# ajzhai/PEANUT

Hardware: AMD Instinct MI355X
Metric: maps/sec for 480x480x(4+N_cat) prediction fwd, batch 32 (higher is better)
Workload: dtype f32; 1 GPU; 480x480, 14-channel (4+10) partial maps -> 6-class prediction forward (PSPNet R50-V1c-D8), batch 32 per GPU, seeded random-init weights; survey_config=2, global_batch=32, parallelism=dp1 (map shards, no data-path collective)

## Files before the change

peanut_amd/csrc/common.h:

```cpp
#pragma once
#include <hip/hip_runtime.h>
#include <stdint.h>
#include <string>

namespace peanut {

void set_error(const std::string& msg);
int fail(int code, const std::string& msg);
void note_kernel(const char* family);
const char* noted_kernel();

#define PEANUT_HIP_CHECK(expr)                                                            \
  do {                                                                                    \
    hipError_t _e = (expr);                                                               \
    if (_e != hipSuccess)                                                                 \
      return ::peanut::fail(-3, std::string(#expr) + ": " + hipGetErrorString(_e));       \
  } while (0)

struct ConvDesc {
  int cin;
  int cout;
  int kh, kw, stride, pad, dil;
  int relu;
  int bn_tile;
// ... 74 lines not shown
bool conv_pw_uses_256w(int cout, long long M, int mt_per_group, int bn_tile, int cin, int flush_ktiles);
bool conv_pw_narrow_tiles(int cin, int cout, long long M, int bn_tile, int mt_per_group);
bool conv_pw_uses_256p(int cout, long long M, int mt_per_group, int bn_tile, int cin, int flush_ktiles, long long in_pixels = 0);
struct ConvKParams;
bool gemm_skinny_takes(const ConvKParams& p, int bn_tile, size_t ws_floats);
int launch_gemm_skinny(const ConvKParams& p, float* ws, size_t ws_floats, hipStream_t stream);
bool conv_pw_uses_256wp(int cout, long long M, int stride, int mt_per_group, int bn_tile, int c1, int c2, int flush_ktiles);
bool conv_pw_uses_ares(int cin, int cout, long long M, int stride, bool two_source, int flush_ktiles, int bn_tile);

bool conv_patch_eligible(const ConvDesc& d, const ConvArgs& a);
const char* conv_patch_kernel_name(const ConvDesc& d, bool nchw);
bool conv_patch_nchw_eligible(const ConvDesc& d, int B, int Ho, int Wo, int creal);
int launch_conv_patch_nchw(const ConvDesc& d, const float* x_nchw, int creal, float* y, int B, int H, int W, int Ho, int Wo, hipStream_t stream);

void wino_geometry(int B, int H, int W, int dil, int* th, int* tw, long long* n_tiles, long long* m_pad, int gran = 128, int m = 4);
void wino_transform_weights(const float* w_oihw, int cout, int cin, float* out, int m = 4);
int launch_wino_input(const float* x, float* V, int B, int H, int W, int C, int dil, hipStream_t s, int gran = 128, int m = 4, long long m_pad_total = 0,
                      const DeferredSplit* df = nullptr);
bool wino_input_accepts_deferred(int B, int H, int W, int C, int dil, int gran, int m);
long long wino_deferred_count();
int launch_wino_output(const float* Mb, const float* scale, const float* shift, const float* res, float* y,
                       int B, int H, int W, int C, int dil, int relu, hipStream_t s, int gran = 128, int m = 4, long long m_pad_total = 0);

bool gemm_rs_uses_256(int cout, long long M, int mt_per_group, int bn_tile, int cin);
const char* gemm_rs_kernel_name(int cout, long long M, int mt_per_group, int bn_tile, int cin, int planes);
size_t sx_packed_bytes(int cin_pad, int cout, int bn_tile, int planes);
void pack_weights_sx(const float* w, int cout, int cin_real, int cin_pad, int bn_tile, int planes, float wscale, void* out);
float sx_pack_scale(const float* w, size_t n, int planes);
size_t sx_conv_packed_bytes(int cin_pad, int cout, int kh, int kw, int bn_tile, int planes);
void pack_weights_sx_conv(const float* w_oihw, int cout, int cin_real, int cin_pad, int kh, int kw, int bn_tile, int planes,
                          float wscale, void* out);

int launch_nchw_to_nhwc_pad(const float* x, float* y, int B, int C, int H, int W, int Cpad, hipStream_t s);
int launch_maxpool3x3s2(const float* x, float* y, int B, int H, int W, int C, int Ho, int Wo, hipStream_t s);
int launch_ppm_pool(const float* x, float* out, int B, int H, int W, int C, const int* scales, int nscales,
                    hipStream_t s, int scale_rows = 0);
size_t ppm_pool_scratch_floats(int B, int H, int C, const int* scales, int nscales);
int launch_ppm_pool2(const float* x, float* scratch, float* out, int B, int H, int W, int C, const int* scales,
                     int nscales, hipStream_t s, int scale_rows = 0);
int launch_ppm_upsample_concat(const float* table, float* out, int B, int H, int W, int Cp, const int* scales,
                               int nscales, int align_corners, hipStream_t s);
int launch_ppm_conv_term(const float* Q, float* R, int B, int H, int W, int C, const int* scales, int nscales,
                         int align_corners, hipStream_t s, int scale_rows = 0);
int launch_upsample_logits(const float* lo, float* out, int B, int h, int w, int K, int H, int W,
                           int align_corners, int sigmoid, hipStream_t s);

// ... 2 lines not shown
```

peanut_amd/csrc/net_common.h:

```cpp
#pragma once
#include <stdlib.h>
#include <math.h>

#include <stdint.h>

#include <map>
#include <memory>
#include <string>
#include <vector>

#include "../../include/peanut_hip.h"
#include "common.h"
#include "options.h"

namespace peanut {

struct DevBuf {
  void* p = nullptr;
  size_t bytes = 0;
  ~DevBuf() { if (p) (void)hipFree(p); }
  int ensure(size_t n) {
    if (n <= bytes) return 0;
    if (p) { (void)hipFree(p); p = nullptr; bytes = 0; }
    hipError_t e = hipMalloc(&p, n);
// ... 43 lines not shown
      if (e2 != hipSuccess) { (void)hipGraphDestroy(g); return fail(PEANUT_EHIP, std::string("hipGraphInstantiate: ") + hipGetErrorString(e2)); }
      hit->graph = g;
      hit->exec = x;
    }
    PEANUT_HIP_CHECK(hipGraphLaunch(hit->exec, s));
    return 0;
  }
};

struct ConvLayer {
  std::string name;
  ConvDesc d{};
  int cin_real = 0;
  DevBuf w, ss;
  bool has_wino = false;
  ConvDesc wino{};
  size_t wino_group_floats = 0;
  DevBuf wino_w, wino_ss;
  DevBuf w_s, wino_w_s;
  size_t wino_group_bytes = 0;
  int wino_m = 4;
  int wino_np() const { return (wino_m + 2) * (wino_m + 2); }
  std::unique_ptr<ConvLayer> alt;
};

inline int rs_planes_of(int precision) {
  return precision == PEANUT_PREC_BF16X6 ? 3 : (precision == PEANUT_PREC_BF16X3 ? 2 : (precision == PEANUT_PREC_FP16X3 ? 4 : 0));
}
inline bool precision_known(int precision) { return precision == PEANUT_PREC_FP32 || rs_planes_of(precision) != 0; }
inline int precision_of_planes(int planes) {
  return planes == 3 ? PEANUT_PREC_BF16X6 : (planes == 2 ? PEANUT_PREC_BF16X3 : (planes == 4 ? PEANUT_PREC_FP16X3 : PEANUT_PREC_FP32));
}
inline bool rs_conv_enabled() {
  return opt(OPT_RS_CONV) != 0;
}
inline int rs_bn_tile(int cin_pad, int cout, int kh, int kw, int pad) {
  if (kh != 1 || kw != 1 || pad != 0 || cin_pad % 16 != 0 || cout < 64) return 0;
  const int bn64_maxk = (int)opt(OPT_RS_BN64_MAXK);
  return (cout >= 128 && cin_pad > bn64_maxk) ? 128 : 64;
}

inline int upload_conv(ConvLayer& L, const float* w_oihw, const float* scale, const float* shift, int cout, int cin,
                int cin_pad, int kh, int kw, int stride, int pad, int dil, int relu, int precision) {
  if (cin_pad % 16 != 0 || cin_pad < cin) return fail(PEANUT_EINVAL, L.name + ": cin_pad must be a multiple of 16 and >= cin");
  ConvDesc& d = L.d;
  d.cin = cin_pad; d.cout = cout; d.kh = kh; d.kw = kw; d.stride = stride; d.pad = pad; d.dil = dil; d.relu = relu;
// ... 117 lines not shown
  g.scale = (const float*)L.wino_ss.p;
  g.shift = (const float*)L.wino_ss.p + g.cout_pad;
  L.wino_group_floats = gf;
  if (g.rs) {
    const size_t gb = sx_packed_bytes(cin_pad, cout, g.bn_tile, g.s_planes);
    std::vector<unsigned char> ps((size_t)np * gb);
    const float wscale = sx_pack_scale(U.data(), U.size(), g.s_planes);
    g.s_alpha = 1.f / wscale;
    for (int pos = 0; pos < np; ++pos)
      pack_weights_sx(U.data() + (size_t)pos * cout * cin, cout, cin, cin_pad, g.bn_tile, g.s_planes, wscale, ps.data() + pos * gb);
    if ((rc = L.wino_w_s.ensure(ps.size()))) return rc;
    PEANUT_HIP_CHECK(hipMemcpy(L.wino_w_s.p, ps.data(), ps.size(), hipMemcpyHostToDevice));
    g.w_s = L.wino_w_s.p;
    L.wino_group_bytes = gb;
  }
  L.has_wino = true;
  return 0;
}

inline int upload_wino_forms(ConvLayer& L, const float* w_oihw, const float* scale, const float* shift, int cout, int cin,
                             int cin_pad, int pad, int dil, int relu, int precision, int requested) {
  int rc;
  if ((rc = upload_wino(L, w_oihw, cout, cin, cin_pad, precision, requested))) return rc;
  if (requested != 0 || L.wino_m != 6) return 0;
  L.alt = std::make_unique<ConvLayer>();
  L.alt->name = L.name;
  if ((rc = upload_conv(*L.alt, w_oihw, scale, shift, cout, cin, cin_pad, 3, 3, 1, pad, dil, relu, precision)) ||
      (rc = upload_wino(*L.alt, w_oihw, cout, cin, cin_pad, precision, 4)))
    return rc;
  if (L.alt->wino_m != 4) { L.alt.reset(); return 0; }
  if (wino5_wanted(dil)) {
    auto& A5 = L.alt->alt;
    A5 = std::make_unique<ConvLayer>();
    A5->name = L.name;
    if ((rc = upload_conv(*A5, w_oihw, scale, shift, cout, cin, cin_pad, 3, 3, 1, pad, dil, relu, precision)) ||
        (rc = upload_wino(*A5, w_oihw, cout, cin, cin_pad, precision, 5)))
      return rc;
  }
  return 0;
}

inline int wino_gran_for(const ConvLayer& L, int B, int H, int W) {
  int th, tw;
  long long n_tiles, m_pad;
  wino_geometry(B, H, W, L.d.dil, &th, &tw, &n_tiles, &m_pad, 256, L.wino_m);
  {
// ... 9 lines not shown
             ? 256 : 128;
}

inline long long wino_padded_rows(const ConvLayer& L, int B, int H, int W) {
  int th, tw;
  long long n_tiles, m_pad;
  wino_geometry(B, H, W, L.d.dil, &th, &tw, &n_tiles, &m_pad, wino_gran_for(L, B, H, W), L.wino_m);
  return (long long)L.wino_np() * m_pad;
}

inline const ConvLayer* wino_pick_form(const ConvLayer* L, int B, int H, int W) {
  if (!L->has_wino || !L->alt || !L->alt->has_wino) return L;
  const ConvLayer* f4 = nullptr;
  const ConvLayer* big = nullptr;
  long long big_rows = 0;
  for (const ConvLayer* c = L; c && c->has_wino; c = c->alt.get()) {
    if (c->wino_m == 4) { f4 = c; continue; }
    const long long r = wino_padded_rows(*c, B, H, W);
    if (!big || r < big_rows || (r == big_rows && c->wino_m < big->wino_m)) { big = c; big_rows = r; }
  }
  if (!f4) return big ? big : L;
  if (!big) return f4;
  return big_rows * 10 <= wino_padded_rows(*f4, B, H, W) * 9 ? big : f4;
}

inline void wino_scratch_floats(const ConvLayer& L, int B, int H, int W, size_t* v, size_t* m) {
  int th, tw;
  long long n_tiles, m_pad;
  wino_geometry(B, H, W, L.d.dil, &th, &tw, &n_tiles, &m_pad, wino_gran_for(L, B, H, W), L.wino_m);
  *v = (size_t)L.wino_np() * m_pad * L.d.cin;
  *m = (size_t)L.wino_np() * m_pad * L.d.cout;
}

inline bool conv_layer_accepts_deferred(const ConvLayer& L, int B, int H, int W) {
  if (!L.has_wino || L.d.rs || L.wino.rs) return false;
  return wino_input_accepts_deferred(B, H, W, L.d.cin, L.d.dil, wino_gran_for(L, B, H, W), L.wino_m);
}

inline int launch_conv_layer(const ConvLayer& L, const ConvArgs& a, float* wino_v, float* wino_m, hipStream_t s, DeferredSplit* produced = nullptr) {
  const bool deferred_in = produced && produced->valid;
  if (!(L.has_wino && !a.x2 && wino_v && wino_m)) {
    if (deferred_in) return fail(PEANUT_EINVAL, L.name + ": the producer deferred its split-K reduce to a layer that cannot sum it");
    return launch_conv(L.d, a, s);
  }
  int th, tw, rc;
  long long n_tiles, m_pad;
// ... 106 lines not shown
```

peanut_amd/csrc/options.h:

```cpp
#pragma once
#include <stdlib.h>
#include <string.h>

#include <string>

namespace peanut {

enum OptionId {
  OPT_PW_GLDS, OPT_PW256_MINK, OPT_PW256_MINTILES, OPT_PW256_PHASE, OPT_PW256_SKIP_PAD, OPT_PW256W_MINK, OPT_PW256W_MINTILES, OPT_PW256P_MINK, OPT_PW256P_MINTILES, OPT_PW256P_FLUSH, OPT_PW256P_ORDER, OPT_PW256P_STREAMK, OPT_PW256WP_MINK, OPT_PW256WP_MINTILES, OPT_PW256WP_NPRE, OPT_PW256WP_STAGGER, OPT_PW_ARES, OPT_PW_SKINNY,
  OPT_PW_ARES_MINUNITS, OPT_PATCH_MINTILES, OPT_STEM_NCHW, OPT_BN64_MAXK, OPT_PW_BN64_MAXK, OPT_PW64_MAXTILES, OPT_FP32_BK, OPT_NCHUNK, OPT_RES_PREFETCH, OPT_SPLIT_MODEL,
  OPT_RS_CONV, OPT_RS_BN64_MAXK, OPT_RS256_MINK, OPT_RS256_MINTILES, OPT_RS64_MAXK, OPT_RS64_MAXTILES,
  OPT_WINO_M, OPT_WINO_HEAD_M, OPT_WINO6_MAXDIL, OPT_WINO5_MINDIL, OPT_WINO_FLUSH_CH, OPT_WINO_MIN_CIN, OPT_WINO_NARROW_MINPIX, OPT_WINO_SMALL_MAXWG, OPT_DEFER_SPLITK,
  OPT_PPM_OVERLAP, OPT_PPM_GROUPED, OPT_PPM_TERM_ROWS, OPT_PPM_GROUP_ROWS, OPT_RCNN_WINO_M, OPT_RCNN_STEM_S2D, OPT_RCNN_RPN_FUSED, OPT_RCNN_FPN_OVERLAP, OPT_RCNN_RANK_SORT, OPT_RCNN_TOPK_SLICE, OPT_RCNN_NMS_LEVELS, OPT_FMM_LOCAL32, OPT_FMM_MAX_PASSES, OPT_FMM_BLOCKED, OPT_FMM_INNER,
  OPT_COUNT
};

struct OptionInfo {
  const char* key;
  long long def;
  bool upload_time;
  const char* help;
};

inline const OptionInfo* option_table() {
  static const OptionInfo t[OPT_COUNT] = {
      {"pw_glds", 1, false, "fp32 1x1 convs / grouped GEMMs on the LDS-DMA kernels of conv_pw.hip (0: conv_igemm)"},
      {"pw256_mink", 1024, false, "fewest input channels for the 256 x 128 three-stage kernel"},
      {"pw256_mintiles", 256, false, "fewest 256 x 128 tiles for that kernel"},
      {"pw256_phase", 1, false, "the two waves of a SIMD request their LDS-DMA pieces half an iteration apart"},
      {"pw256_skip_pad", 1, false, "256 x 128 kernel, grouped GEMMs: waves whose rows are all group padding issue no MFMAs (0: compute the zero rows)"},
      {"pw256w_mink", 768, false, "fewest input channels for the 256 x 256 two-stage kernel (0: off)"},
      {"pw256w_mintiles", 1536, false, "fewest 256 x 256 tiles for that kernel"},
      {"pw256p_mink", 512, false, "fewest input channels for the persistent 256 x 128 kernel (conv_pw256p.hip; 0: off)"},
      {"pw256p_mintiles", 512, false, "fewest 256 x 128 tiles for that kernel"},
      {"pw256p_flush", 512, false, "most input channels of a Winograd position GEMM (two-level accumulation) that runs on the persistent kernel (0: none)"},
// ... 9 lines not shown
      {"patch_mintiles", 1024, false, "3x3 convs of 16 / 32 input channels on the persistent LDS-patch kernel (conv_patch.hip) from this many 8 x 16 output tiles (0: off)"},
      {"stem_nchw", 1, false, "prediction forward: the first stem conv reads the NCHW input itself (conv_patch.hip, NCHW variant) instead of a layout pass + NHWC conv (fp32 mode, when the patch kernel takes the layer)"},
      {"bn64_maxk", 256, true, "128 x 64 tiles for layers with at most this many input channels"},
      {"pw_bn64_maxk", 128, true, "pointwise layers / Winograd position GEMMs: weights PACKED 64 wide up to this many input channels (wider layers: 128-wide packing, 64-wide tiles chosen per shape)"},
      {"pw64_maxtiles", 512, false, "a 128-wide-packed pointwise layer with at most bn64_maxk input channels runs 128 x 64 tiles while its 128 x 128 tiling has fewer tiles than this (two per CU)"},
      {"fp32_bk", 0, true, "16: force 16-channel k-tiles in conv_igemm (experiment)"},
      {"nchunk", 8, false, "n-tiles per chunk of the tile order (0: n fastest over all n-tiles)"},
      {"res_prefetch", 1, false, "request the first residual rows before the last k-tile's MFMAs"},
      {"split_model", 1, false, "tail split-K plan counts CUs (1) or resident slots (0)"},
      {"rs_conv", 1, true, "emulated modes: non-pointwise convs on conv_rs.hip (0: fp32 MFMA kernel)"},
      {"rs_bn64_maxk", 128, true, "emulated modes: 128 x 64 tiles up to this many input channels"},
      {"rs256_mink", 512, false, "emulated modes: fewest input channels for the 256 x 256 kernel"},
      {"rs256_mintiles", 256, false, "emulated modes: fewest 256 x 256 tiles for it"},
      {"rs64_maxk", 512, false, "emulated modes: 64 x 64 tiles up to this many input channels"},
      {"rs64_maxtiles", 128, false, "emulated modes: ... and below this many 128-row tiles"},
      {"wino_m", 0, true, "4 / 5 / 6: force one Winograd form on every eligible layer (0: policy)"},
      {"wino_head_m", 0, true, "4 / 5 / 6: Winograd form of the PSP bottleneck (0: policy)"},
      {"wino6_maxdil", 4, true, "largest dilation that gets an F(6x6) form"},
      {"wino5_mindil", 4, true, "smallest dilation that also gets an F(5x5) form (0: none)"},
      {"wino_flush_ch", 64, true, "channels per partial sum of the position GEMMs' two-level accumulation (0: off)"},
      {"wino_min_cin", 0, true, "fewest input channels of a Winograd layer (0: the planner's policy)"},
      {"wino_narrow_minpix", 20000, false, "layers under 128 channels take their Winograd form from this many input pixels on (round 6: 100 000 -> 20 000 -- with the small-problem transforms one 720 x 720 map's layer1 conv2, 32 400 pixels, gains 5 us per layer as F(6x6); profiles/r9e)"},
      {"wino_small_maxwg", 1024, false, "Winograd transforms: launches with fewer workgroups than this of the one-thread-per-tile kernels take the small-problem variants (a workgroup per tile and 64-channel slice, a thread per line, through LDS; bit-identical; 0: never)"},
      {"defer_splitk", 1, false, "a Bottleneck conv1 whose every tile is split along k leaves its partial tiles unsummed and conv2's (small-problem) Winograd input transform sums them: one launch fewer per block at batch 1, bit-identical (0: every conv runs its own reduce); read when a (B, H, W) plan is built"},
      {"ppm_overlap", -1, false, "pyramid branch of the PSP head on a side stream: 0 / 1, -1 = by size"},
      {"ppm_grouped", -1, false, "per-scale PSP GEMMs as one grouped launch: 0 / 1, -1 = by size"},
      {"ppm_term_rows", 1, false, "folded pyramid term: one wave per output row, no barrier in the row loop (0: the workgroup-wide two-phase kernel)"},
      {"ppm_group_rows", 0, false, "pyramid pooling, row pass: rows added up per workgroup (1..5; 0 = by size: as many as still leave ~768 workgroups)"},
      {"rcnn_wino_m", 0, true, "detector front end: 4 / 5 / 6 pins one Winograd form (0: per shape)"},
      {"rcnn_stem_s2d", 1, true, "detector stem 7x7 stride 2 as a space-to-depth 4x4 conv"},
      {"rcnn_rpn_fused", 1, false, "detector: the RPN head on all five pyramid levels as one chain (five input transforms, ONE grouped Winograd GEMM, five output transforms, one objectness and one anchor-delta GEMM over all levels' rows: 12 launches instead of 25); read when a (B, H, W) plan is built"},
      {"rcnn_fpn_overlap", 0, false, "detector: the FPN output convs of p5, p4, p3 on a side stream next to the lateral / top-down chain that ends in p2's (round 5 experiment, bit-identical; measured SLOWER at batch 1, 5.70 against 5.61 ms per frame, profiles/r8: off); read when a (B, H, W) plan is built"},
      {"rcnn_rank_sort", 1, false, "detector: the RPN candidates of an image are ordered by counting the larger keys (n / 64 workgroups) instead of one workgroup's bitonic sort (round 5; same order: the keys are distinct)"},
      {"rcnn_topk_slice", 20480, false, "detector: objectness logits per workgroup of the per-level top-k (a level is cut into up to 8 ranges whose k largest are merged by counting; 0: one workgroup per level, round 4)"},
      {"rcnn_nms_levels", 1, false, "detector: the proposal NMS level by level (five 16 x 16-word suppression blocks and five scans per image side by side, post-NMS top-k by counting) instead of one score-sorted list per image (round 5; same proposals)"},
      {"fmm_local32", 1, false, "goal solver: single-precision local solve inside a tile"},
      {"fmm_max_passes", 24, false, "goal solver: hard ceiling of the second-order ordering passes; they stop as soon as a pass changes nothing (6-10 passes on the agent's 960 x 960 map; peanut_goal_converged reports whether they reached their fixed point)"},
      {"fmm_blocked", 1, false, "goal solver: a wave relaxes its 8 x 8 block of the tile to convergence between workgroup barriers (round 5; 0: one Jacobi sweep of the whole tile per barrier pair)"},
      {"fmm_inner", 48, false, "goal solver: iterations a wave spends on its block before it publishes it (blocked rounds)"},
  };
  return t;
}

struct Options {
  long long v[OPT_COUNT];
};
// ... 48 lines not shown
```

peanut_amd/csrc/pred_api.hip:

```cpp
#include <math.h>
#include <string.h>

#include <map>
#include <memory>
#include <string>
#include <vector>

#include "net_common.h"

namespace peanut {

static thread_local std::string g_err;
void set_error(const std::string& msg) { g_err = msg; }
int fail(int code, const std::string& msg) {
  g_err = msg;
  return code;
}
static thread_local const char* g_kernel = "";
void note_kernel(const char* family) { g_kernel = family; }
const char* noted_kernel() { return g_kernel; }

namespace {

enum OpKind { OP_TO_NHWC, OP_CONV, OP_CONV_NCHW, OP_MAXPOOL, OP_PPM_POOL, OP_PPM_UP, OP_PPM_TERM, OP_UPSAMPLE, OP_WINO_IN, OP_WINO_GEMM, OP_WINO_OUT };

struct Op {
  OpKind kind;
  std::string name;
  std::string kernel;
  const ConvLayer* conv = nullptr;
  Act in, in2, res, out;
  bool has_in2 = false, has_res = false;
  double flops = 0;
  double bytes = 0;
  int wino_mt_per_group = 0;
  int wino_valid_rows = 0;
  int wino_gran = 128;
  int branch = 0;
  bool fork_before = false, join_before = false;
  int group_mt = 0;
  int ppm_scale_rows = 0;
  bool defer_ok = false;
};

struct Plan {
  int B = 0, H = 0, W = 0;
  Act splitk;
// ... 149 lines not shown
    a.B = out->B; a.Ho = out->H; a.Wo = out->W;
    if (conv_patch_eligible(d, a)) return conv_patch_kernel_name(d, false);
  }
  if (d.rs == 2) return std::string(d.s_planes == 3 ? "conv_rs6_128x" : (d.s_planes == 4 ? "conv_rs3h_128x" : "conv_rs3_128x")) + std::to_string(d.bn_tile);
  if (d.rs) return gemm_rs_kernel_name(d.cout, M, mt_per_group, d.bn_tile, d.cin, d.s_planes);
  if (d.bk == 32 && d.kh == 1 && d.kw == 1 && d.pad == 0 && (!two_source || d.stride == 1) && d.cin % 32 == 0 && conv_pw_enabled())
  {
    const int flush = d.flush_ch / d.bk;
    if (conv_pw_uses_256wp(d.cout, M, d.stride, mt_per_group, d.bn_tile, d.cin, 0, flush))
      return "conv_pw_glds_256x256p";
    if (conv_pw_uses_ares(d.cin, d.cout, M, d.stride, two_source, flush, d.bn_tile)) return "conv_pw_ares_128x128";
    if (conv_pw_uses_256w(d.cout, M, mt_per_group, d.bn_tile, d.cin, flush)) return "conv_pw_glds_256x256";
    if (conv_pw_uses_256p(d.cout, M, mt_per_group, d.bn_tile, d.cin, flush, M * d.stride * d.stride)) return "conv_pw_glds_256x128p";
    if (conv_pw_uses_256(d.cout, M, mt_per_group, d.bn_tile, d.cin)) return "conv_pw_glds_256x128";
    if (conv_pw_narrow_tiles(d.cin, d.cout, M, d.bn_tile, mt_per_group)) return "conv_pw_glds_128x64";
    return "conv_pw_glds_128x" + std::to_string(d.bn_tile);
  }
  return "conv_igemm_128x" + std::to_string(d.bn_tile) + "x" + std::to_string(d.bk);
}

void push_conv(Plan& pl, const ConvLayer* L, const Act& in, const Act* in2, const Act* res, const Act& out, Arena* ar = nullptr) {
  const bool wino = L->has_wino && !in2 && ar && (long long)in.B * in.H * in.W >= wino_min_pixels(L->d.cin);
  if (wino) L = wino_pick_form(L, in.B, in.H, in.W);
  if (wino) {
    int th, tw;
    long long n_tiles, m_pad;
    const bool rs_gemm = L->wino.rs != 0;
    const int gran = wino_gran_for(*L, in.B, in.H, in.W);
    wino_geometry(in.B, in.H, in.W, L->d.dil, &th, &tw, &n_tiles, &m_pad, gran, L->wino_m);
    const double np = (double)L->wino_np();
    const long long npl = L->wino_np();
    Act v = make_act(*ar, 1, 1, (int)(npl * m_pad), in.C);
    Act m = make_act(*ar, 1, 1, (int)(npl * m_pad), L->d.cout);
    const std::string fam = L->wino_m == 6 ? "wino6_" : (L->wino_m == 5 ? "wino5_" : "wino_");
    const std::string tag = "[" + fam;
    Op a; a.kind = OP_WINO_IN; a.name = L->name + tag + "in]"; a.kernel = fam + "input"; a.conv = L; a.in = in; a.out = v;
    a.wino_gran = gran;
    a.bytes = (double)in.bytes + np * (double)n_tiles * in.C * 4.0;
    pl.ops.push_back(a);
    Op g; g.kind = OP_WINO_GEMM; g.name = L->name + tag + "gemm]"; g.kernel = conv_kernel_name(L->wino, false, npl * m_pad, (int)(m_pad / 128)); g.conv = L;
    g.in = v; g.in.W = (int)(npl * m_pad); g.in.C = in.C; g.out = m; g.wino_mt_per_group = (int)(m_pad / 128); g.wino_gran = gran; g.wino_valid_rows = (int)n_tiles;
    g.flops = 2.0 * np * (double)m_pad * L->d.cout * L->cin_real;
    g.bytes = np * (double)m_pad * (in.C * 4.0 + L->d.cout * 4.0) +
              np * (rs_gemm ? (double)L->wino_group_bytes : (double)L->wino_group_floats * 4);
    pl.ops.push_back(g);
    Op o; o.kind = OP_WINO_OUT; o.name = L->name + tag + "out]"; o.kernel = fam + "output"; o.conv = L; o.in = m; o.out = out;
// ... 61 lines not shown
    Act y = make_act(ar, B, conv_out_dim(x.H, 3, 2, 1, 1), conv_out_dim(x.W, 3, 2, 1, 1), x.C);
    Op op; op.kind = OP_MAXPOOL; op.name = "maxpool"; op.kernel = "maxpool"; op.in = x; op.out = y;
    op.bytes = (double)x.bytes + (double)y.bytes;
    pl->ops.push_back(op);
    pl->named["pool"] = y;
    rel(x);
    x = y;
  }
  for (size_t li = 0; li < h->layers.size(); ++li) {
    for (size_t bi = 0; bi < h->layers[li].size(); ++bi) {
      const auto& blk = h->layers[li][bi];
      const ConvDesc& d2 = blk.c2->d;
      Act t1 = make_act(ar, B, x.H, x.W, blk.c1->d.cout);
      push_conv(*pl, blk.c1, x, nullptr, nullptr, t1);
      const int h2 = conv_out_dim(x.H, 3, d2.stride, d2.pad, d2.dil), w2 = conv_out_dim(x.W, 3, d2.stride, d2.pad, d2.dil);
      Act t2 = make_act(ar, B, h2, w2, d2.cout);
      const size_t c1_idx = pl->ops.size() - 1;
      push_conv(*pl, blk.c2, t1, nullptr, nullptr, t2, &ar);
      {
        const Op& win = pl->ops[c1_idx + 1];
        if (opt(OPT_DEFER_SPLITK) != 0 && !h->keep_all && win.kind == OP_WINO_IN && pl->ops[c1_idx].kind == OP_CONV && !win.conv->d.rs &&
            wino_input_accepts_deferred(t1.B, t1.H, t1.W, t1.C, win.conv->d.dil, win.wino_gran, win.conv->wino_m))
          pl->ops[c1_idx].defer_ok = true;
      }
      rel(t1);
      Act idn = x;
      bool own_idn = false;
      const bool fused_c3d = blk.c3d != nullptr && !h->keep_all;
      if (blk.down && !fused_c3d) {
        idn = make_act(ar, B, h2, w2, blk.down->d.cout);
        push_conv(*pl, blk.down, x, nullptr, nullptr, idn);
        own_idn = true;
      }
      Act y = make_act(ar, B, h2, w2, blk.c3->d.cout);
      if (fused_c3d) push_conv(*pl, blk.c3d, t2, &x, nullptr, y);
      else push_conv(*pl, blk.c3, t2, nullptr, &idn, y);
      rel(t2);
      if (own_idn) rel(idn);
      rel(x);
      x = y;
    }
    pl->named["layer" + std::to_string(li + 1)] = x;
  }
  const int overlap_env = (int)opt(OPT_PPM_OVERLAP);
  const bool overlap = h->bottleneck_x != nullptr && (overlap_env >= 0 ? overlap_env == 1 : (long long)B * x.H * x.W >= 4096);
  const size_t side_first = pl->ops.size();
// ... 185 lines not shown
      }
      if (op.defer_ok) a.defer = &h->deferred;
      return launch_conv(op.conv->d, a, s);
    }
    case OP_WINO_IN: {
      const int rc = launch_wino_input(P(op.in), P(op.out), op.in.B, op.in.H, op.in.W, op.in.C, op.conv->d.dil, s, op.wino_gran, op.conv->wino_m, 0,
                                       h->deferred.valid ? &h->deferred : nullptr);
      h->deferred.valid = false;
      return rc;
    }
    case OP_WINO_GEMM: {
      ConvArgs a{};
      a.x = P(op.in); a.y = P(op.out);
      a.B = 1; a.H = 1; a.W = op.in.W; a.c1 = op.in.C; a.c2 = 0; a.Ho = 1; a.Wo = op.in.W;
      a.ws = P(op.branch ? pl.splitk2 : pl.splitk); a.ws_floats = kSplitKScratchFloats;
      a.mt_per_group = op.wino_mt_per_group;
      a.group_valid_rows = op.wino_valid_rows;
      a.w_group_stride = op.conv->wino.rs ? op.conv->wino_group_bytes : op.conv->wino_group_floats;
      return launch_conv(op.conv->wino, a, s);
    }
    case OP_WINO_OUT:
      return launch_wino_output(P(op.in), op.conv->d.scale, op.conv->d.shift, op.has_res ? P(op.res) : nullptr, P(op.out),
                                op.out.B, op.out.H, op.out.W, op.out.C, op.conv->d.dil, op.conv->d.relu, s, op.wino_gran, op.conv->wino_m);
    case OP_MAXPOOL:
      return launch_maxpool3x3s2(P(op.in), P(op.out), op.in.B, op.in.H, op.in.W, op.in.C, op.out.H, op.out.W, s);
    case OP_PPM_POOL:
      return launch_ppm_pool2(P(op.in), op.has_in2 ? P(op.in2) : nullptr, P(op.out), op.in.B, op.in.H, op.in.W, op.in.C,
                              h->cfg.pool_scales, h->cfg.n_pool_scales, s, op.ppm_scale_rows);
    case OP_PPM_UP:
      return launch_ppm_upsample_concat(P(op.in), P(op.out), op.out.B, op.out.H, op.out.W, h->cfg.head_channels,
                                        h->cfg.pool_scales, h->cfg.n_pool_scales, h->cfg.align_corners, s);
    case OP_PPM_TERM:
      return launch_ppm_conv_term(P(op.in), P(op.out), op.out.B, op.out.H, op.out.W, h->cfg.head_channels,
                                  h->cfg.pool_scales, h->cfg.n_pool_scales, h->cfg.align_corners, s, op.ppm_scale_rows);
    case OP_UPSAMPLE:
      return launch_upsample_logits(P(op.in), out_dev, op.in.B, op.in.H, op.in.W, op.in.C, pl.H, pl.W,
                                    h->cfg.align_corners, sigmoid, s);
  }
  return fail(PEANUT_EINVAL, "unknown op");
}

extern "C" {

const char* peanut_last_error(void) { return g_err.c_str(); }
const char* peanut_last_conv_kernel(void) { return noted_kernel(); }
int peanut_abi_version(void) { return 15; }
// ... 389 lines not shown
```

peanut_amd/csrc/winograd.hip:

```cpp
#include <stdlib.h>

#include <atomic>

#include "common.h"
#include "conv_common.h"

namespace peanut {

namespace {

template <typename V>
__device__ __forceinline__ V fmak(V a, float k, V c) { return __builtin_elementwise_fma(a, (V)k, c); }

__device__ __forceinline__ void bt6(const f32x4 d0, const f32x4 d1, const f32x4 d2, const f32x4 d3, const f32x4 d4,
                                    const f32x4 d5, f32x4& t0, f32x4& t1, f32x4& t2, f32x4& t3, f32x4& t4, f32x4& t5) {
#pragma clang fp contract(off)
  const f32x4 a = fmak(d2, -2.25f, d4), b = fmak(d3, 0.75f, -1.6875f * d1);
  const f32x4 c = fmak(d2, -0.5625f, d4), e = fmak(d3, 1.5f, -0.84375f * d1);
  t0 = fmak(d0, 1.265625f, fmak(d2, -2.8125f, d4));
  t1 = a + b;
  t2 = a - b;
  t3 = c + e;
  t4 = c - e;
  t5 = fmak(d1, 1.265625f, fmak(d3, -2.8125f, d5));
// ... 630 lines not shown
#pragma unroll
    for (int k = 0; k < 4; ++k) {
      const int r = r0 + k * g.d;
      const bool ok = c < g.W && r < g.H;
      const size_t off = ok ? (img + (size_t)r * g.W + c) * g.C + ng * 4 : 0;
      rc[k] = *reinterpret_cast<const f32x4*>(res + off);
    }
  }
  const f32x4 sc = *reinterpret_cast<const f32x4*>(scale + ng * 4);
  const f32x4 sh = *reinterpret_cast<const f32x4*>(shift + ng * 4);
  f32x4 o0, o1, o2, o3;
  at6(qs[0][a][l], qs[1][a][l], qs[2][a][l], qs[3][a][l], qs[4][a][l], qs[5][a][l], o0, o1, o2, o3);
  if (c >= g.W) return;
  const f32x4 o[4] = {o0, o1, o2, o3};
#pragma unroll
  for (int k = 0; k < 4; ++k) {
    const int r = r0 + k * g.d;
    if (r >= g.H) continue;
    const size_t off = (img + (size_t)r * g.W + c) * g.C + ng * 4;
    f32x4 v = o[k] * sc + sh;
    if constexpr (RES) v += rc[k];
    if (relu) v = relu_keep_nan(v);
    *reinterpret_cast<f32x4*>(y + off) = v;
  }
}

int wino_small_lanes(long long n_tiles, int C, int m) {
  const long long maxwg = opt(OPT_WINO_SMALL_MAXWG);
  if (maxwg <= 0 || (m != 4 && m != 6)) return 0;
  const long long big_wgs = (n_tiles * (m == 4 ? C / 4 : C / 2) + 255) / 256;
  if (big_wgs >= maxwg) return 0;
  const int per32 = m == 4 ? 128 : 64, per16 = per32 / 2;
  const int lanes = C % per32 == 0 ? 32 : (C % per16 == 0 ? 16 : 0);
  if (!lanes || n_tiles * (C / (lanes * (m == 4 ? 4 : 2))) > 0x7fffffffLL) return 0;
  return lanes;
}

int grid_for(long long total) {
  long long blocks = (total + 255) / 256;
  if (blocks > 256LL * 64) blocks = 256LL * 64;
  if (blocks < 1) blocks = 1;
  return (int)blocks;
}

}

// ... 71 lines not shown
  }
  if (const int lanes = wino_small_lanes(g.n_tiles, C, m)) {
    const unsigned grid = (unsigned)(g.n_tiles * (C / (lanes * (m == 4 ? 4 : 2))));
#define PEANUT_WINO_SMALL_IN(K, L, T)                                                                          \
    do {                                                                                                       \
      if (defer && src.split_p == 4) hipLaunchKernelGGL((K<L, 4>), dim3(grid), dim3(T), 0, s, x, V, g, src);   \
      else if (defer && src.split_p == 2) hipLaunchKernelGGL((K<L, 2>), dim3(grid), dim3(T), 0, s, x, V, g, src); \
      else if (defer) hipLaunchKernelGGL((K<L, 0>), dim3(grid), dim3(T), 0, s, x, V, g, src);                  \
      else hipLaunchKernelGGL((K<L, -1>), dim3(grid), dim3(T), 0, s, x, V, g, src);                            \
    } while (0)
    if (m == 6 && lanes == 32) PEANUT_WINO_SMALL_IN(wino6_input_small_kernel, 32, 256);
    else if (m == 6) PEANUT_WINO_SMALL_IN(wino6_input_small_kernel, 16, 128);
    else if (lanes == 32) PEANUT_WINO_SMALL_IN(wino4_input_small_kernel, 32, 192);
    else PEANUT_WINO_SMALL_IN(wino4_input_small_kernel, 16, 96);
#undef PEANUT_WINO_SMALL_IN
  } else if (m == 6) hipLaunchKernelGGL(wino6_input_kernel, dim3(grid_for(total)), dim3(256), 0, s, x, V, g);
  else if (m == 5) hipLaunchKernelGGL(wino5_input_kernel, dim3(grid_for(total)), dim3(256), 0, s, x, V, g);
  else hipLaunchKernelGGL(wino_input_kernel, dim3(grid_for(total)), dim3(256), 0, s, x, V, g);
  hipError_t e = hipGetLastError();
  if (e != hipSuccess) return fail(-3, std::string("wino_input launch: ") + hipGetErrorString(e));
  return 0;
}

int launch_wino_output(const float* Mb, const float* scale, const float* shift, const float* res, float* y,
                       int B, int H, int W, int C, int dil, int relu, hipStream_t s, int gran, int m, long long m_pad_total) {
  if (C % 4 || m < 4 || m > 6) return fail(-2, "wino_output: channels must be a multiple of 4, tiles 4x4, 5x5 or 6x6");
  WinoGeom g{B, H, W, C, dil, 0, 0, 0, 0};
  wino_geometry(B, H, W, dil, &g.th, &g.tw, &g.n_tiles, &g.m_pad, gran, m);
  if (m_pad_total > 0) g.m_pad = m_pad_total;
  const long long total = g.n_tiles * (m == 4 ? C / 4 : C / 2);
  if (const int lanes = wino_small_lanes(g.n_tiles, C, m)) {
    const unsigned grid = (unsigned)(g.n_tiles * (C / (lanes * (m == 4 ? 4 : 2))));
#define PEANUT_WINO_SMALL_OUT(K, R, L, T) hipLaunchKernelGGL((K<R, L>), dim3(grid), dim3(T), 0, s, Mb, scale, shift, res, y, g, relu)
    if (m == 6 && lanes == 32) { if (res) PEANUT_WINO_SMALL_OUT(wino6_output_small_kernel, true, 32, 256); else PEANUT_WINO_SMALL_OUT(wino6_output_small_kernel, false, 32, 256); }
    else if (m == 6) { if (res) PEANUT_WINO_SMALL_OUT(wino6_output_small_kernel, true, 16, 128); else PEANUT_WINO_SMALL_OUT(wino6_output_small_kernel, false, 16, 128); }
    else if (lanes == 32) { if (res) PEANUT_WINO_SMALL_OUT(wino4_output_small_kernel, true, 32, 192); else PEANUT_WINO_SMALL_OUT(wino4_output_small_kernel, false, 32, 192); }
    else { if (res) PEANUT_WINO_SMALL_OUT(wino4_output_small_kernel, true, 16, 96); else PEANUT_WINO_SMALL_OUT(wino4_output_small_kernel, false, 16, 96); }
#undef PEANUT_WINO_SMALL_OUT
  } else if (m == 6 && res) hipLaunchKernelGGL(wino6_output_kernel<true>, dim3(grid_for(total)), dim3(256), 0, s, Mb, scale, shift, res, y, g, relu);
  else if (m == 6) hipLaunchKernelGGL(wino6_output_kernel<false>, dim3(grid_for(total)), dim3(256), 0, s, Mb, scale, shift, res, y, g, relu);
  else if (m == 5) hipLaunchKernelGGL(wino5_output_kernel, dim3(grid_for(total)), dim3(256), 0, s, Mb, scale, shift, res, y, g, relu);
  else if (res) hipLaunchKernelGGL(wino_output_kernel<true>, dim3(grid_for(total)), dim3(256), 0, s, Mb, scale, shift, res, y, g, relu);
  else hipLaunchKernelGGL(wino_output_kernel<false>, dim3(grid_for(total)), dim3(256), 0, s, Mb, scale, shift, res, y, g, relu);
  hipError_t e = hipGetLastError();
  if (e != hipSuccess) return fail(-3, std::string("wino_output launch: ") + hipGetErrorString(e));
  return 0;
// ... 4 lines not shown
```

Baseline: 886.6 maps/s.

## Fuse F(6x6) Winograd transforms and GEMM into one kernel for 64-channel layers

Adds a single kernel for the 64->64 channel F(6x6) Winograd convolutions (layer1 conv2) that runs the input transform, the per-position MFMA GEMMs and the output transform with BN/ReLU in one pass. Intermediate V and M tensors stay in LDS and registers instead of going through global memory, and two launches are removed. The trade-off is weights re-read per workgroup from global/L2, 512-thread blocks with large register accumulators that may limit occupancy, and extra syncs per chunk. It is enabled by default for layers without a residual and with at least 4096 tiles.

```diff
diff --git a/peanut_amd/csrc/common.h b/peanut_amd/csrc/common.h
--- a/peanut_amd/csrc/common.h
+++ b/peanut_amd/csrc/common.h
@@ -120,6 +120,10 @@
 int launch_wino_output(const float* Mb, const float* scale, const float* shift, const float* res, float* y,
                        int B, int H, int W, int C, int dil, int relu, hipStream_t s, int gran = 128, int m = 4, long long m_pad_total = 0);
 
+void wino6_fused_pack_weights(const float* U, float* out);
+int launch_wino6_fused(const float* x, const float* wf, const float* scale, const float* shift, float* y, int B, int H, int W, int C,
+                       int relu, hipStream_t s);
+
 bool gemm_rs_uses_256(int cout, long long M, int mt_per_group, int bn_tile, int cin);
 const char* gemm_rs_kernel_name(int cout, long long M, int mt_per_group, int bn_tile, int cin, int planes);
 size_t sx_packed_bytes(int cin_pad, int cout, int bn_tile, int planes);
diff --git a/peanut_amd/csrc/net_common.h b/peanut_amd/csrc/net_common.h
--- a/peanut_amd/csrc/net_common.h
+++ b/peanut_amd/csrc/net_common.h
@@ -89,6 +89,7 @@
   int wino_m = 4;
   int wino_np() const { return (wino_m + 2) * (wino_m + 2); }
   std::unique_ptr<ConvLayer> alt;
+  DevBuf wino_fused_w;
 };
 
 inline int rs_planes_of(int precision) {
@@ -252,6 +253,13 @@
                              int cin_pad, int pad, int dil, int relu, int precision, int requested) {
   int rc;
   if ((rc = upload_wino(L, w_oihw, cout, cin, cin_pad, precision, requested))) return rc;
+  if (L.wino_m == 6 && !L.wino.rs && !L.d.rs && dil == 1 && cin == 64 && cin_pad == 64 && cout == 64) {
+    std::vector<float> U((size_t)64 * cout * cin), packed((size_t)64 * cout * cin);
+    wino_transform_weights(w_oihw, cout, cin, U.data(), 6);
+    wino6_fused_pack_weights(U.data(), packed.data());
+    if ((rc = L.wino_fused_w.ensure(packed.size() * sizeof(float)))) return rc;
+    PEANUT_HIP_CHECK(hipMemcpy(L.wino_fused_w.p, packed.data(), packed.size() * sizeof(float), hipMemcpyHostToDevice));
+  }
   if (requested != 0 || L.wino_m != 6) return 0;
   L.alt = std::make_unique<ConvLayer>();
   L.alt->name = L.name;
@@ -307,6 +315,14 @@
   if (!f4) return big ? big : L;
   if (!big) return f4;
   return big_rows * 10 <= wino_padded_rows(*f4, B, H, W) * 9 ? big : f4;
+}
+
+inline bool wino_fused_takes(const ConvLayer& L, int B, int H, int W, bool res) {
+  if (opt(OPT_WINO_FUSED) == 0 || !L.wino_fused_w.p || L.wino_m != 6 || res) return false;
+  int th, tw;
+  long long n_tiles, m_pad;
+  wino_geometry(B, H, W, 1, &th, &tw, &n_tiles, &m_pad, 128, 6);
+  return n_tiles >= 4096;
 }
 
 inline void wino_scratch_floats(const ConvLayer& L, int B, int H, int W, size_t* v, size_t* m) {
diff --git a/peanut_amd/csrc/options.h b/peanut_amd/csrc/options.h
--- a/peanut_amd/csrc/options.h
+++ b/peanut_amd/csrc/options.h
@@ -10,7 +10,7 @@
   OPT_PW_GLDS, OPT_PW256_MINK, OPT_PW256_MINTILES, OPT_PW256_PHASE, OPT_PW256_SKIP_PAD, OPT_PW256W_MINK, OPT_PW256W_MINTILES, OPT_PW256P_MINK, OPT_PW256P_MINTILES, OPT_PW256P_FLUSH, OPT_PW256P_ORDER, OPT_PW256P_STREAMK, OPT_PW256WP_MINK, OPT_PW256WP_MINTILES, OPT_PW256WP_NPRE, OPT_PW256WP_STAGGER, OPT_PW_ARES, OPT_PW_SKINNY,
   OPT_PW_ARES_MINUNITS, OPT_PATCH_MINTILES, OPT_STEM_NCHW, OPT_BN64_MAXK, OPT_PW_BN64_MAXK, OPT_PW64_MAXTILES, OPT_FP32_BK, OPT_NCHUNK, OPT_RES_PREFETCH, OPT_SPLIT_MODEL,
   OPT_RS_CONV, OPT_RS_BN64_MAXK, OPT_RS256_MINK, OPT_RS256_MINTILES, OPT_RS64_MAXK, OPT_RS64_MAXTILES,
-  OPT_WINO_M, OPT_WINO_HEAD_M, OPT_WINO6_MAXDIL, OPT_WINO5_MINDIL, OPT_WINO_FLUSH_CH, OPT_WINO_MIN_CIN, OPT_WINO_NARROW_MINPIX, OPT_WINO_SMALL_MAXWG, OPT_DEFER_SPLITK,
+  OPT_WINO_M, OPT_WINO_HEAD_M, OPT_WINO6_MAXDIL, OPT_WINO5_MINDIL, OPT_WINO_FLUSH_CH, OPT_WINO_MIN_CIN, OPT_WINO_NARROW_MINPIX, OPT_WINO_SMALL_MAXWG, OPT_WINO_FUSED, OPT_DEFER_SPLITK,
   OPT_PPM_OVERLAP, OPT_PPM_GROUPED, OPT_PPM_TERM_ROWS, OPT_PPM_GROUP_ROWS, OPT_RCNN_WINO_M, OPT_RCNN_STEM_S2D, OPT_RCNN_RPN_FUSED, OPT_RCNN_FPN_OVERLAP, OPT_RCNN_RANK_SORT, OPT_RCNN_TOPK_SLICE, OPT_RCNN_NMS_LEVELS, OPT_FMM_LOCAL32, OPT_FMM_MAX_PASSES, OPT_FMM_BLOCKED, OPT_FMM_INNER,
   OPT_COUNT
 };
@@ -66,6 +66,7 @@
       {"wino_min_cin", 0, true, "fewest input channels of a Winograd layer (0: the planner's policy)"},
       {"wino_narrow_minpix", 20000, false, "layers under 128 channels take their Winograd form from this many input pixels on (round 6: 100 000 -> 20 000 -- with the small-problem transforms one 720 x 720 map's layer1 conv2, 32 400 pixels, gains 5 us per layer as F(6x6); profiles/r9e)"},
       {"wino_small_maxwg", 1024, false, "Winograd transforms: launches with fewer workgroups than this of the one-thread-per-tile kernels take the small-problem variants (a workgroup per tile and 64-channel slice, a thread per line, through LDS; bit-identical; 0: never)"},
+      {"wino_fused", 1, false, "fp32 prediction plans: the 64 -> 64 channel F(6x6) layers (layer1 conv2) of launches with at least 4096 tiles as ONE kernel -- transforms and position GEMMs fused, V / M never in memory (winograd.hip: wino6_fused64_kernel; 0: input transform, grouped GEMM, output transform); read when a (B, H, W) plan is built"},
       {"defer_splitk", 1, false, "a Bottleneck conv1 whose every tile is split along k leaves its partial tiles unsummed and conv2's (small-problem) Winograd input transform sums them: one launch fewer per block at batch 1, bit-identical (0: every conv runs its own reduce); read when a (B, H, W) plan is built"},
       {"ppm_overlap", -1, false, "pyramid branch of the PSP head on a side stream: 0 / 1, -1 = by size"},
       {"ppm_grouped", -1, false, "per-scale PSP GEMMs as one grouped launch: 0 / 1, -1 = by size"},
diff --git a/peanut_amd/csrc/pred_api.hip b/peanut_amd/csrc/pred_api.hip
--- a/peanut_amd/csrc/pred_api.hip
+++ b/peanut_amd/csrc/pred_api.hip
@@ -22,7 +22,7 @@
 
 namespace {
 
-enum OpKind { OP_TO_NHWC, OP_CONV, OP_CONV_NCHW, OP_MAXPOOL, OP_PPM_POOL, OP_PPM_UP, OP_PPM_TERM, OP_UPSAMPLE, OP_WINO_IN, OP_WINO_GEMM, OP_WINO_OUT };
+enum OpKind { OP_TO_NHWC, OP_CONV, OP_CONV_NCHW, OP_MAXPOOL, OP_PPM_POOL, OP_PPM_UP, OP_PPM_TERM, OP_UPSAMPLE, OP_WINO_IN, OP_WINO_GEMM, OP_WINO_OUT, OP_WINO_FUSED };
 
 struct Op {
   OpKind kind;
@@ -218,6 +218,16 @@
 void push_conv(Plan& pl, const ConvLayer* L, const Act& in, const Act* in2, const Act* res, const Act& out, Arena* ar = nullptr) {
   const bool wino = L->has_wino && !in2 && ar && (long long)in.B * in.H * in.W >= wino_min_pixels(L->d.cin);
   if (wino) L = wino_pick_form(L, in.B, in.H, in.W);
+  if (wino && wino_fused_takes(*L, in.B, in.H, in.W, res != nullptr)) {
+    int th, tw;
+    long long n_tiles, m_pad;
+    wino_geometry(in.B, in.H, in.W, 1, &th, &tw, &n_tiles, &m_pad, 16, 6);
+    Op op; op.kind = OP_WINO_FUSED; op.name = L->name + "[wino6_fused]"; op.kernel = "wino6_fused"; op.conv = L; op.in = in; op.out = out;
+    op.flops = 2.0 * 64 * (double)m_pad * L->d.cout * L->cin_real;
+    op.bytes = (double)in.bytes + (double)out.bytes + (double)L->wino_fused_w.bytes;
+    pl.ops.push_back(op);
+    return;
+  }
   if (wino) {
     int th, tw;
     long long n_tiles, m_pad;
@@ -325,6 +335,10 @@
         if (opt(OPT_DEFER_SPLITK) != 0 && !h->keep_all && win.kind == OP_WINO_IN && pl->ops[c1_idx].kind == OP_CONV && !win.conv->d.rs &&
             wino_input_accepts_deferred(t1.B, t1.H, t1.W, t1.C, win.conv->d.dil, win.wino_gran, win.conv->wino_m))
           pl->ops[c1_idx].defer_ok = true;
+      }
+      if (pl->keep_all) {
+        pl->named[blk.c1->name] = t1;
+        pl->named[blk.c2->name] = t2;
       }
       rel(t1);
       Act idn = x;
@@ -556,6 +570,9 @@
     case OP_WINO_OUT:
       return launch_wino_output(P(op.in), op.conv->d.scale, op.conv->d.shift, op.has_res ? P(op.res) : nullptr, P(op.out),
                                 op.out.B, op.out.H, op.out.W, op.out.C, op.conv->d.dil, op.conv->d.relu, s, op.wino_gran, op.conv->wino_m);
+    case OP_WINO_FUSED:
+      return launch_wino6_fused(P(op.in), (const float*)op.conv->wino_fused_w.p, op.conv->d.scale, op.conv->d.shift, P(op.out),
+                                op.in.B, op.in.H, op.in.W, op.in.C, op.conv->d.relu, s);
     case OP_MAXPOOL:
       return launch_maxpool3x3s2(P(op.in), P(op.out), op.in.B, op.in.H, op.in.W, op.in.C, op.out.H, op.out.W, s);
     case OP_PPM_POOL:
diff --git a/peanut_amd/csrc/winograd.hip b/peanut_amd/csrc/winograd.hip
--- a/peanut_amd/csrc/winograd.hip
+++ b/peanut_amd/csrc/winograd.hip
@@ -676,6 +676,115 @@
     if constexpr (RES) v += rc[k];
     if (relu) v = relu_keep_nan(v);
     *reinterpret_cast<f32x4*>(y + off) = v;
+  }
+}
+
+constexpr int kFusedC = 64;
+constexpr int kFusedChunk = 16;
+constexpr int kFusedChunks = kFusedC / kFusedChunk;
+constexpr int kFusedTiles = 16;
+
+__global__ __launch_bounds__(512) void wino6_fused64_kernel(const float* __restrict__ x, const float* __restrict__ wf,
+                                                           const float* __restrict__ scale, const float* __restrict__ shift,
+                                                           float* __restrict__ y, const WinoGeom g, int relu) {
+  __shared__ f32x4 u[8][8][4][kFusedTiles];
+  const int lane = threadIdx.x & 63, wave = threadIdx.x >> 6;
+  const int t = lane & 15, q = lane >> 4;
+  const long long tile = (long long)blockIdx.x * kFusedTiles + t;
+  const bool tok = tile < g.n_tiles;
+  int b = 0, oy, ox, ty = 0, tx = 0;
+  if (tok) decode_tile(g, tile, b, oy, ox, ty, tx);
+  const int r0 = 6 * ty - 1, col = 6 * tx - 1 + wave;
+  const bool cok = tok && (unsigned)col < (unsigned)g.W;
+  const float* xb = x + (size_t)b * g.H * g.W * kFusedC + 4 * q;
+  auto load_column = [&](int k, f32x4 (&p)[8]) __attribute__((always_inline)) {
+#pragma unroll
+    for (int i = 0; i < 8; ++i) {
+      const int r = r0 + i;
+      f32x4 v = {0.f, 0.f, 0.f, 0.f};
+      if (cok && (unsigned)r < (unsigned)g.H) v = *reinterpret_cast<const f32x4*>(xb + ((size_t)r * g.W + col) * kFusedC + k * kFusedChunk);
+      p[i] = v;
+    }
+  };
+  f32x4 acc[8][4];
+#pragma unroll
+  for (int j = 0; j < 8; ++j)
+#pragma unroll
+    for (int nb = 0; nb < 4; ++nb) acc[j][nb] = f32x4{0.f, 0.f, 0.f, 0.f};
+  f32x4 pf[8];
+  load_column(0, pf);
+  const float* wp = wf + (size_t)wave * 8 * kFusedChunks * 4 * 256 + lane * 4;
+  for (int k = 0; k < kFusedChunks; ++k) {
+    __syncthreads();
+    {
+      f32x2 lo[8], hi[8];
+#pragma unroll
+      for (int i = 0; i < 8; ++i) { lo[i] = pf[i].xy; hi[i] = pf[i].zw; }
+      bt8(lo[0], lo[1], lo[2], lo[3], lo[4], lo[5], lo[6], lo[7], lo[0], lo[1], lo[2], lo[3], lo[4], lo[5], lo[6], lo[7]);
+      bt8(hi[0], hi[1], hi[2], hi[3], hi[4], hi[5], hi[6], hi[7], hi[0], hi[1], hi[2], hi[3], hi[4], hi[5], hi[6], hi[7]);
+#pragma unroll
+      for (int i = 0; i < 8; ++i) u[i][wave][q][t] = f32x4{lo[i].x, lo[i].y, hi[i].x, hi[i].y};
+    }
+    __syncthreads();
+    f32x4 v[8];
+    {
+      f32x2 lo[8], hi[8];
+#pragma unroll
+      for (int j = 0; j < 8; ++j) { const f32x4 s = u[wave][j][q][t]; lo[j] = s.xy; hi[j] = s.zw; }
+      f32x2 tl[8], th[8];
+      bt8(lo[0], lo[1], lo[2], lo[3], lo[4], lo[5], lo[6], lo[7], tl[0], tl[1], tl[2], tl[3], tl[4], tl[5], tl[6], tl[7]);
+      bt8(hi[0], hi[1], hi[2], hi[3], hi[4], hi[5], hi[6], hi[7], th[0], th[1], th[2], th[3], th[4], th[5], th[6], th[7]);
+#pragma unroll
+      for (int j = 0; j < 8; ++j) v[j] = f32x4{tl[j].x, tl[j].y, th[j].x, th[j].y};
+    }
+    if (k + 1 < kFusedChunks) load_column(k + 1, pf);
+    const float* wk = wp + (size_t)k * 4 * 256;
+#pragma unroll
+    for (int j = 0; j < 8; ++j) {
+      f32x4 w[4];
+#pragma unroll
+      for (int nb = 0; nb < 4; ++nb) w[nb] = *reinterpret_cast<const f32x4*>(wk + ((size_t)j * kFusedChunks * 4 + nb) * 256);
+#pragma unroll
+      for (int s = 0; s < 4; ++s)
+#pragma unroll
+        for (int nb = 0; nb < 4; ++nb) acc[j][nb] = __builtin_amdgcn_mfma_f32_16x16x4f32(w[nb][s], v[j][s], acc[j][nb], 0, 0, 0);
+    }
+  }
+  const int orow = 6 * ty, ocol = 6 * tx + wave;
+  const size_t img = (size_t)b * g.H * g.W;
+#pragma unroll
+  for (int nb = 0; nb < 4; ++nb) {
+    f32x2 ql[6], qh[6];
+    {
+      f32x2 ml[8], mh[8];
+#pragma unroll
+      for (int j = 0; j < 8; ++j) { ml[j] = acc[j][nb].xy; mh[j] = acc[j][nb].zw; }
+      at8(ml[0], ml[1], ml[2], ml[3], ml[4], ml[5], ml[6], ml[7], ql[0], ql[1], ql[2], ql[3], ql[4], ql[5]);
+      at8(mh[0], mh[1], mh[2], mh[3], mh[4], mh[5], mh[6], mh[7], qh[0], qh[1], qh[2], qh[3], qh[4], qh[5]);
+    }
+    __syncthreads();
+#pragma unroll
+    for (int a = 0; a < 6; ++a) u[wave][a][q][t] = f32x4{ql[a].x, ql[a].y, qh[a].x, qh[a].y};
+    __syncthreads();
+    if (wave < 6 && tok && ocol < g.W) {
+      f32x2 ml[8], mh[8];
+#pragma unroll
+      for (int i = 0; i < 8; ++i) { const f32x4 s = u[i][wave][q][t]; ml[i] = s.xy; mh[i] = s.zw; }
+      f32x2 ol[6], oh[6];
+      at8(ml[0], ml[1], ml[2], ml[3], ml[4], ml[5], ml[6], ml[7], ol[0], ol[1], ol[2], ol[3], ol[4], ol[5]);
+      at8(mh[0], mh[1], mh[2], mh[3], mh[4], mh[5], mh[6], mh[7], oh[0], oh[1], oh[2], oh[3], oh[4], oh[5]);
+      const int n = nb * 16 + 4 * q;
+      const f32x2 scl = *reinterpret_cast<const f32x2*>(scale + n), sch = *reinterpret_cast<const f32x2*>(scale + n + 2);
+      const f32x2 shl = *reinterpret_cast<const f32x2*>(shift + n), shh = *reinterpret_cast<const f32x2*>(shift + n + 2);
+#pragma unroll
+      for (int kr = 0; kr < 6; ++kr) {
+        const int r = orow + kr;
+        if (r >= g.H) continue;
+        f32x2 vl = ol[kr] * scl + shl, vh = oh[kr] * sch + shh;
+        if (relu) { vl.x = relu_keep_nan(vl.x); vl.y = relu_keep_nan(vl.y); vh.x = relu_keep_nan(vh.x); vh.y = relu_keep_nan(vh.y); }
+        *reinterpret_cast<f32x4*>(y + (img + (size_t)r * g.W + ocol) * kFusedC + n) = f32x4{vl.x, vl.y, vh.x, vh.y};
+      }
+    }
   }
 }
 
@@ -793,6 +902,31 @@
   return 0;
 }
 
+void wino6_fused_pack_weights(const float* U, float* out) {
+  const int C = kFusedC;
+  for (int p = 0; p < 64; ++p)
+    for (int k = 0; k < kFusedChunks; ++k)
+      for (int nb = 0; nb < C / 16; ++nb)
+        for (int l = 0; l < 64; ++l)
+          for (int s = 0; s < 4; ++s) {
+            const int n = nb * 16 + (l & 15), c = k * kFusedChunk + 4 * (l >> 4) + s;
+            out[((((size_t)p * kFusedChunks + k) * (C / 16) + nb) * 64 + l) * 4 + s] = U[((size_t)p * C + n) * C + c];
+          }
+}
+
+int launch_wino6_fused(const float* x, const float* wf, const float* scale, const float* shift, float* y, int B, int H, int W, int C,
+                       int relu, hipStream_t s) {
+  if (C != kFusedC) return fail(-2, "wino6_fused: 64 input and output channels only");
+  WinoGeom g{B, H, W, C, 1, 0, 0, 0, 0};
+  wino_geometry(B, H, W, 1, &g.th, &g.tw, &g.n_tiles, &g.m_pad, 128, 6);
+  const long long items = (g.n_tiles + kFusedTiles - 1) / kFusedTiles;
+  if (items > 0x7fffffffLL) return fail(-2, "wino6_fused: problem too large");
+  hipLaunchKernelGGL(wino6_fused64_kernel, dim3((unsigned)items), dim3(512), 0, s, x, wf, scale, shift, y, g, relu);
+  hipError_t e = hipGetLastError();
+  if (e != hipSuccess) return fail(-3, std::string("wino6_fused launch: ") + hipGetErrorString(e));
+  return 0;
+}
+
 int launch_wino_output(const float* Mb, const float* scale, const float* shift, const float* res, float* y,
                        int B, int H, int W, int C, int dil, int relu, hipStream_t s, int gran, int m, long long m_pad_total) {
   if (C % 4 || m < 4 || m > 6) return fail(-2, "wino_output: channels must be a multiple of 4, tiles 4x4, 5x5 or 6x6");
```

Result: no change. 889.3 maps/s, median of 6 (+0.3%).
